# KLab/YAIK

Measured on AMD Instinct MI355X. Metric: Mpix/s tile encode (alpha reject + 7 gradient passes + 8x8 range quant), 8K RGBA, higher is better.
Workload: dtype u8/int32 (+f32 mode-selection sums)

## Files before the change

yaik_amd/csrc/yk_encode2.hip:

```cpp
#include "yk_common.h"
#include "yk_curves.h"
#include "yk_device.h"
#include <mutex>

__constant__ float c_curve2[6][16] = YK_CURVE_TABLE;

#define LS YK_LSTRIDE
#ifdef YK_TEST_HOOKS
#define YK2_ABLATE(bit) ((P.ablate & (bit)) != 0)
#else
#define YK2_ABLATE(bit) false
#endif

__device__ __forceinline__ int y2_byte(uint32_t w, int ch) { return (w >> (8 * ch)) & 255; }
__device__ __forceinline__ uint32_t y2_absdiff(uint32_t a, uint32_t b) { uint32_t r; asm("v_sad_u32 %0, %1, %2, 0" : "=v"(r) : "v"(a), "v"(b)); return r; }
__device__ __forceinline__ int y2_round6(int v) { return (v & ~3) | (v >> 6); }
__device__ __forceinline__ int y2_round6p(int v) { v = min(v + 1, 255); return (v & ~3) | (v >> 6); }

typedef short y2s2 __attribute__((ext_vector_type(2)));
typedef unsigned short y2u2 __attribute__((ext_vector_type(2)));
__device__ __forceinline__ y2u2 y2_u2(uint32_t w) { return __builtin_bit_cast(y2u2, w); }
__device__ __forceinline__ y2s2 y2_s2(y2u2 v) { return __builtin_bit_cast(y2s2, v); }
__device__ __forceinline__ y2u2 y2_splat(int v) { const unsigned short t = (unsigned short)v; return (y2u2){ t, t }; }
__device__ __forceinline__ y2s2 y2_splats(int v) { const short t = (short)v; return (y2s2){ t, t }; }
// ... 283 lines not shown
        const y2s2 rA = __builtin_elementwise_max(__builtin_elementwise_sub_sat(W.loR, mnA), __builtin_elementwise_sub_sat(mxA, W.hiR));
        unsigned long long f = y2_fold<NX, NY>(__ballot(oA.x > 0));
        f &= y2_fold<NX, NY>(__ballot(oA.y > 0));
        f &= y2_fold<NX, NY>(__ballot(rA.x > 0));
        f &= y2_fold<NX, NY>(__ballot(rA.y > 0));
        return f;
    };
    auto failP2 = [&](const y2s2 mnP, const y2s2 mxP) -> unsigned long long {
        const y2s2 oP = __builtin_elementwise_max(__builtin_elementwise_sub_sat(W.loO, mnP), __builtin_elementwise_sub_sat(mxP, W.hiO));
        const y2s2 rP = __builtin_elementwise_max(__builtin_elementwise_sub_sat(W.loR, mnP), __builtin_elementwise_sub_sat(mxP, W.hiR));
        return y2_fold<NX, NY>(__ballot((oP.x > 0) | (oP.y > 0))) & y2_fold<NX, NY>(__ballot((rP.x > 0) | (rP.y > 0)));
    };
    auto mnAll = [&]() { return __builtin_elementwise_min(__builtin_elementwise_min(mn[0], mn[1]), mn[2]); };
    auto mxAll = [&]() { return __builtin_elementwise_max(__builtin_elementwise_max(mx[0], mx[1]), mx[2]); };

    constexpr bool kScreen = (NX * NY >= 4);
    constexpr unsigned kA = 0x07u, kP = 0x18u;
    unsigned long long accept;
    if (SMOOTH) {
        setup(0); setup(1); setup(2);
        pixelRow(0, kA, true);
        nextRow(0, kA); pixelRow(1, kA, false);
        nextRow(1, kA); pixelRow(2, kA, false);
        nextRow(2, kA); pixelRow(3, kA, false);
        YK2_STAT(kPassId * 10 + 4, 1);
        accept = viable & ~failA4(mnAll(), mxAll());
        const unsigned long long rest = viable & ~accept;
        if (rest != 0ULL) {
            YK2_STAT(kPassId * 10 + 5, 1); YK2_STAT(90 + kPassId, __popcll(y2_spread<NX, NY>(rest)));
            setup(3);
            pixelRow(0, 0x08u, true);
            const unsigned long long left = rest & ~failP2(mn[3], mx[3]);
            if (left != 0ULL) {
                setup(4);
                pixelRow(0, 0x10u, true);
                nextRow(0, kP); pixelRow(1, kP, false);
                nextRow(1, kP); pixelRow(2, kP, false);
                nextRow(2, kP); pixelRow(3, kP, false);
                accept |= left & ~failP2(__builtin_elementwise_min(mn[3], mn[4]), __builtin_elementwise_max(mx[3], mx[4]));
            }
        }
    } else {
        if (kScreen) {
            setup(0); setup(3);
            pixelRow(0, 0x09u, true);
            viable &= ~(failA4(mn[0], mx[0]) & failP2(mn[3], mx[3]));
            if (viable == 0ULL) { YK2_STAT(kPassId * 10 + 2, 1); return 0ULL; }
            setup(1); setup(2);
            pixelRow(0, 0x06u, true);
            viable &= ~(failA4(mnAll(), mxAll()) & failP2(mn[3], mx[3]));
            if (viable == 0ULL) { YK2_STAT(kPassId * 10 + 3, 1); return 0ULL; }
            nextRow(0, kA);
            pixelRow(1, kA, false);
        } else {
#pragma unroll
            for (int t = 0; t < 5; t++) setup(t);
            pixelRow(0, 0x1Fu, true);
            viable &= ~(failA4(mnAll(), mxAll()) & failP2(__builtin_elementwise_min(mn[3], mn[4]), __builtin_elementwise_max(mx[3], mx[4])));
            if (viable == 0ULL) { YK2_STAT(kPassId * 10 + 3, 1); return 0ULL; }
            nextRow(0, 0x1Fu);
            pixelRow(1, 0x1Fu, false);
            if (NX * NY <= 2) {
                viable &= ~(failA4(mnAll(), mxAll()) & failP2(__builtin_elementwise_min(mn[3], mn[4]), __builtin_elementwise_max(mx[3], mx[4])));
                if (viable == 0ULL) { YK2_STAT(kPassId * 10 + 9, 1); return 0ULL; }
            }
        }
        YK2_STAT(kPassId * 10 + 4, 1);
        nextRow(1, kA);
        pixelRow(2, kA, false);
        nextRow(2, kA);
        pixelRow(3, kA, false);
        accept = viable & ~failA4(mnAll(), mxAll());
        const unsigned long long rest = viable & ~accept;
        if (rest != 0ULL) {
            YK2_STAT(kPassId * 10 + 5, 1); YK2_STAT(90 + kPassId, __popcll(y2_spread<NX, NY>(rest)));
            if (kScreen) {
                setup(4);
                pixelRow(0, 0x10u, true);
                nextRow(0, kP);
                pixelRow(1, kP, false);
            }
            nextRow(1, kP);
            pixelRow(2, kP, false);
            nextRow(2, kP);
            pixelRow(3, kP, false);
            accept |= rest & ~failP2(__builtin_elementwise_min(mn[3], mn[4]), __builtin_elementwise_max(mx[3], mx[4]));
        }
    }
    return accept;
}

template <int SX, int SY, bool SMOOTH = false>
__device__ __forceinline__ void y2_grad_pass(const Y2Pass pass, unsigned long long& cov, unsigned long long& evaluated) {
    constexpr int NX = (1 << SX) / 4, NY = (1 << SY) / 4, kPassId = y2_pass_id<SX, SY>();
    const int lane = pass.lane;
    const unsigned long long viable = y2_viable<SX, SY>(pass, cov) & ~evaluated;
    evaluated = 0ULL;
    if (viable == 0ULL) return;
    YK2_STAT(kPassId * 10 + 0, 1); YK2_STAT(kPassId * 10 + 8, __popcll(y2_spread<NX, NY>(viable)));
    if (y2_compact_sweep<SX, SY>(pass, viable, cov, evaluated)) return;
    const unsigned long long accept = y2_full_pass<SX, SY, SMOOTH>(pass, viable);
    if (accept == 0ULL) return;
    YK2_STAT(kPassId * 10 + 6, 1);
    y2_accept<SX, SY>(pass, cov, accept);
}

#define YK2_QROWS 258
#define YK2_QR0 32
#define YK2_QNR 224
#define YK2_QBYTES ((size_t)YK2_QNR * YK2_QROWS * 16)
#define YK2_RCPBYTES ((size_t)256 * sizeof(float))
#define YK2_DEFN1 224
#define YK2_DEFBYTES ((size_t)225 * YK2_DEFN1 * 4)
#define YK2_TABBYTES (YK2_QBYTES + YK2_RCPBYTES + YK2_DEFBYTES)
typedef _Float16 y2h2 __attribute__((ext_vector_type(2)));
__device__ __forceinline__ uint32_t y2_f16_bits(int n) { const _Float16 h = (_Float16)(float)n; return (uint32_t)__builtin_bit_cast(unsigned short, h); }
__global__ void yk_qtab_kernel(uint4* tab) {
    __shared__ int K[6][16];
    const int R = YK2_QR0 + (int)blockIdx.x, t = threadIdx.x;
    if (t < 96) { const int m = t >> 4, i = t & 15; K[m][i] = __float2int_rz(__fmul_rn(c_curve2[m][i], (float)R)); }
    __syncthreads();
    if (t < YK2_QROWS) {
        const int o = t - 2;
        uint32_t md[6], idx = 0;
        for (int m = 0; m < 6; m++) {
            const int cnt = m < 3 ? 16 : 8;
            int best = 1 << 30, bi = 0;
            for (int n = 0; n < cnt; n++) { const int d = abs(K[m][n] - o); if (d < best) { best = d; bi = n; } }
            best = min(best, 255);
            md[m] = y2_f16_bits(best);
            idx |= (uint32_t)bi << (4 * m);
        }
        tab[(size_t)blockIdx.x * YK2_QROWS + t] = make_uint4(md[0] | (md[1] << 16), md[2] | (md[3] << 16), md[4] | (md[5] << 16), idx);
    }
}
struct Y2TileDef { int base, BN, dist, R; };
__device__ __forceinline__ Y2TileDef y2_tile_def(const int min_, const int d8) {
    Y2TileDef d;
    d.base = (min_ * 63 + 112) / 224;
    d.BN = (d.base * 224) / 63;
    const int scale = 223 - d.BN;
    const int dnum = (d8 - 32) * 127 + (scale - 1);
    d.dist = (scale < 0) ? -dnum : dnum / scale;
    d.R = (d.dist * scale) / 127 + 32;
    return d;
}
__global__ void yk_deftab_kernel(uint32_t* tab) {
    const int min_ = blockIdx.x, d8 = 32 + (int)threadIdx.x;
    const Y2TileDef d = y2_tile_def(min_, d8);
    const int R = min(max(d.R, YK2_QR0), YK2_QR0 + YK2_QNR - 1);
    const uint32_t rowBase = (uint32_t)((R - YK2_QR0) * YK2_QROWS + 2 - d.BN + 256);
    tab[min_ * YK2_DEFN1 + (int)threadIdx.x] = rowBase | (((((uint32_t)d.dist & 255u) << 7) | ((uint32_t)d.base & 255u)) << 16);
}

__global__ void yk_selftest_qtab_kernel(const uint4* tab, const uint32_t* deftab, int* mismatches) {
    const int mn = blockIdx.x, mx = threadIdx.x;
    if (mx < mn) return;
    const int min_ = min(mn, 224);
    int diff = mx - min_; if (diff < 16) diff = 16;
    const int d8 = max(diff, 32);
    const Y2TileDef d = y2_tile_def(min_, d8);
    const int BN = d.BN, R = d.R;
    int bad = 0;
    if (R < YK2_QR0 || R >= YK2_QR0 + YK2_QNR || mn - BN < -2) { atomicAdd(mismatches, 1); return; }
    {
        const uint32_t e = deftab[min_ * YK2_DEFN1 + (d8 - 32)];
        if ((e & 0xFFFFu) != (uint32_t)((R - YK2_QR0) * YK2_QROWS + 2 - BN + 256)) bad++;
        if ((e >> 16) != ((((uint32_t)d.dist & 255u) << 7) | ((uint32_t)d.base & 255u))) bad++;
    }
    for (int m = 0; m < 6; m++) {
        const int cnt = m < 3 ? 16 : 8;
        int L[16];
        for (int i = 0; i < cnt; i++) {
            L[i] = __float2int_rz(__fadd_rn((float)BN, __fmul_rn(c_curve2[m][i], (float)R)));
            if (L[i] != BN + __float2int_rz(__fmul_rn(c_curve2[m][i], (float)R))) bad++;
        }
        for (int v = mn; v <= mx; v++) {
            int best = 1 << 30, bi = 0;
            for (int n = 0; n < cnt; n++) { const int dd = abs(L[n] - v); if (dd < best) { best = dd; bi = n; } }
            const uint4 row = tab[(size_t)(R - YK2_QR0) * YK2_QROWS + (v - BN + 2)];
            const uint32_t w = m < 2 ? row.x : (m < 4 ? row.y : row.z);
            const uint32_t hb = (m & 1) ? (w >> 16) : (w & 0xFFFFu);
            const int ix = (row.w >> (4 * m)) & 15;
            if (hb != y2_f16_bits(best) || ix != bi) bad++;
        }
    }
    if (bad) atomicAdd(mismatches, bad);
}

#define YK2_RUN 16
template <int K> __device__ __forceinline__ uint32_t y2_writelane_k(uint32_t v, uint32_t old) { asm("v_writelane_b32 %0, %1, %2" : "+v"(old) : "s"(v), "n"(K)); return old; }
__device__ __forceinline__ uint32_t y2_writelane(uint32_t v, int k, uint32_t old) {
    switch (k) {
        case 0: return y2_writelane_k<0>(v, old); case 1: return y2_writelane_k<1>(v, old); case 2: return y2_writelane_k<2>(v, old);
        case 3: return y2_writelane_k<3>(v, old); case 4: return y2_writelane_k<4>(v, old); case 5: return y2_writelane_k<5>(v, old);
        case 11: return y2_writelane_k<11>(v, old); default: return y2_writelane_k<12>(v, old);
    }
}
#ifdef YK2_TIMING
__device__ unsigned long long g_y2_times[65536 * 16];
#define YK2_PROBE(i) do { if ((i) == 0 && lane == 0 && unit < 65536) { g_y2_times[(size_t)unit * 16 + 10] = 0; g_y2_times[(size_t)unit * 16 + 11] = 0; g_y2_times[(size_t)unit * 16 + 12] = y2_t_entry; g_y2_times[(size_t)unit * 16 + 13] = ((unsigned long long)y2_xcc << 32) | y2_hwid; } if (lane == 0 && unit < 65536) { g_y2_times[(size_t)unit * 16 + 2 * (i)] = __builtin_amdgcn_s_memtime(); g_y2_times[(size_t)unit * 16 + 2 * (i) + 1] = __builtin_amdgcn_s_memrealtime(); } } while (0)
extern "C" int yk_debug_wave_times(unsigned long long* out) { return (int)hipMemcpyFromSymbol(out, HIP_SYMBOL(g_y2_times), sizeof(g_y2_times)); }
#else
#define YK2_PROBE(i) do { } while (0)
#endif
#define YK2_LUTW 84
#ifndef YK2_WIN
#define YK2_WIN 16
#endif
#ifndef YK2_PREF
#define YK2_PREF 8
#endif
#ifndef YK2_RVWIN
#define YK2_RVWIN 8
#endif

#define Y2_QUAD_X 0xB1
#define Y2_QUAD_Y 0x4E
template <int CTRL> __device__ __forceinline__ int y2_quad(int v) { return __builtin_amdgcn_update_dpp(v, v, CTRL, 0xF, 0xF, true); }
template <int CTRL> __device__ __forceinline__ float y2_quad(float v) { return __int_as_float(y2_quad<CTRL>(__float_as_int(v))); }
template <int FIRST> __device__ __forceinline__ void y2_quad_sums(float (&t)[6]) {
#define Y2_QX(i) "v_add_f32_dpp %" #i ", %" #i ", %" #i " quad_perm:[1,0,3,2] row_mask:0xf bank_mask:0xf\n\t"
#define Y2_QY(i) "v_add_f32_dpp %" #i ", %" #i ", %" #i " quad_perm:[2,3,0,1] row_mask:0xf bank_mask:0xf\n\t"
    if (FIRST == 0)
        asm volatile("s_nop 1\n\t" Y2_QX(0) Y2_QX(1) Y2_QX(2) Y2_QX(3) Y2_QX(4) Y2_QX(5) Y2_QY(0) Y2_QY(1) Y2_QY(2) Y2_QY(3) Y2_QY(4) Y2_QY(5)
                     : "+v"(t[0]), "+v"(t[1]), "+v"(t[2]), "+v"(t[3]), "+v"(t[4]), "+v"(t[5]));
    else
        asm volatile("s_nop 1\n\t" Y2_QX(0) Y2_QX(1) Y2_QX(2) Y2_QY(0) Y2_QY(1) Y2_QY(2) : "+v"(t[3]), "+v"(t[4]), "+v"(t[5]));
#undef Y2_QX
#undef Y2_QY
}
__device__ __forceinline__ float y2_row16_sum(float x) {
    x = __fadd_rn(x, y2_quad<Y2_QUAD_X>(x));
    x = __fadd_rn(x, y2_quad<Y2_QUAD_Y>(x));
    x = __fadd_rn(x, __int_as_float(__builtin_amdgcn_update_dpp(0, __float_as_int(x), 0x141, 0xF, 0xF, true)));
    x = __fadd_rn(x, __int_as_float(__builtin_amdgcn_update_dpp(0, __float_as_int(x), 0x140, 0xF, 0xF, true)));
    return x;
}
__device__ __forceinline__ uint32_t y2_byte_x4(uint32_t w, int ch) {
    uint32_t r; const uint32_t two = 2u;
    if (ch == 0) asm("v_lshlrev_b32_sdwa %0, %1, %2 dst_sel:DWORD dst_unused:UNUSED_PAD src0_sel:DWORD src1_sel:BYTE_0" : "=v"(r) : "v"(two), "v"(w));
    else if (ch == 1) asm("v_lshlrev_b32_sdwa %0, %1, %2 dst_sel:DWORD dst_unused:UNUSED_PAD src0_sel:DWORD src1_sel:BYTE_1" : "=v"(r) : "v"(two), "v"(w));
    else asm("v_lshlrev_b32_sdwa %0, %1, %2 dst_sel:DWORD dst_unused:UNUSED_PAD src0_sel:DWORD src1_sel:BYTE_2" : "=v"(r) : "v"(two), "v"(w));
    return r;
}
__device__ __forceinline__ void y2_fma_lo(float& acc, uint32_t h, float w) { asm volatile("v_fma_mix_f32 %0, %1, %2, %0 op_sel_hi:[1,0,0]" : "+v"(acc) : "v"(h), "v"(w)); }
__device__ __forceinline__ void y2_fma_hi(float& acc, uint32_t h, float w) { asm volatile("v_fma_mix_f32 %0, %1, %2, %0 op_sel:[1,0,0] op_sel_hi:[1,0,0]" : "+v"(acc) : "v"(h), "v"(w)); }
__device__ __forceinline__ uint32_t y2_pack3(int r, int g, int b) {
    return __builtin_amdgcn_perm((uint32_t)b, __builtin_amdgcn_perm((uint32_t)g, (uint32_t)r, 0x0C0C0400u), 0x0C040100u);
}

template <bool WANT_DST, bool MODE3>
__global__ __launch_bounds__(64, 4) void yk_encode2_kernel(const YkEncodeParams P) {
    constexpr int kStart = MODE3 ? 3 : 0;
    constexpr int kPixWords = 17 * LS, kLutWords = WANT_DST ? 16 * YK2_LUTW : 0;
    __shared__ __attribute__((aligned(16))) uint32_t s_mem[kPixWords > kLutWords ? kPixWords : kLutWords];
    uint32_t* const s_pix = s_mem;
    uint32_t (*const s_lut)[YK2_LUTW] = reinterpret_cast<uint32_t (*)[YK2_LUTW]>(s_mem);
    __shared__ uint32_t s_bm[24];
    __shared__ uint8_t s_list[64];
    __shared__ __attribute__((aligned(16))) float s_curve[WANT_DST ? 6 : 1][16];
    __shared__ __attribute__((aligned(16))) float s_rcp[256];
    __shared__ __attribute__((aligned(16))) uint32_t s_aux[432];
    uint32_t* const s_lat = s_aux;
    float (*const s_chain)[68] = reinterpret_cast<float (*)[68]>(s_aux);
    float* const s_err = reinterpret_cast<float*>(s_aux + 408);
    __shared__ uint32_t s_range[3 * 64];
    __shared__ __attribute__((aligned(16))) uint32_t s_sp[3 * 4 * 8 + 3 * 4 * 16];

    uint32_t* const s_tile = s_aux + 416;
    __shared__ uint32_t s_iwTest[WANT_DST ? 1024 : 1];
    uint32_t* const s_iw = WANT_DST ? s_iwTest : s_mem;
    uint32_t* const s_park = WANT_DST ? s_iwTest : s_sp;
    static_assert(WANT_DST || kPixWords >= 1024, "index words need 4 KB");

    const int lane = threadIdx.x;
    __builtin_amdgcn_s_setprio(3);
#ifdef YK2_TIMING
    const unsigned long long y2_t_entry = __builtin_amdgcn_s_memrealtime();
    const unsigned y2_hwid = __builtin_amdgcn_s_getreg((4 << 0) | (0 << 6) | (31 << 11)), y2_xcc = __builtin_amdgcn_s_getreg((20 << 0) | (0 << 6) | (31 << 11));
#endif
    typedef const __attribute__((address_space(4))) YkEncodeParams* Y2ParamPtr;
    auto strip = [&](const int slot, const int xcd, const int lane, Y2ParamPtr const Pp) {
    const __attribute__((address_space(4))) YkEncodeParams& P = *Pp;
    const int nBf = P.xBB64 * P.yBB64, nB = nBf * P.nFrames;
    const int grp = slot / (YK2_RUN * 4);
    const int unit = (grp * 8 + ((xcd + grp) & 7)) * (YK2_RUN * 4) + (slot - grp * (YK2_RUN * 4));
    int L = unit >> 2; const int wave = unit & 3;
    const bool spare = L >= nB;
    L = spare ? 0 : L;
    const uint32_t frU = yk_udiv((uint32_t)L, P.divNBf.mul, P.divNBf.shift);
    L -= (int)frU * nBf;
    const size_t fr = frU;
    const int32_t* const pl0 = P.plane[0] + fr * P.fs.plane; const int32_t* const pl1 = P.plane[1] + fr * P.fs.plane; const int32_t* const pl2 = P.plane[2] + fr * P.fs.plane;
    const int BY = (int)yk_udiv((uint32_t)L, P.divXBB64.mul, P.divXBB64.shift), BX = L - BY * P.xBB64;
    const int w = P.w, h = P.h;
    const int mt0 = (BY * 4 + wave) * P.mtW + BX * 4;

    YK2_PROBE(0);
    if (lane < 24) s_bm[lane] = 0;
    typedef uint32_t y2_u32x2 __attribute__((ext_vector_type(2)));
    typedef int32_t y2_i32x4 __attribute__((ext_vector_type(4)));
    y2_u32x2 keep8; y2_i32x4 bnd;
    {
        const int g4 = (lane & 15) * 4, r0 = lane >> 4;
        const int gx = BX * 64 + g4;
        const bool inX = gx + 3 < w;
        const int gxc = min(gx, w - 4);
        const int gyS = BY * 64 + wave * 16;
        const int gyB = min(gyS, P.hAvail - 1);
        const size_t rowBase = (size_t)gyB * (size_t)P.strideElems;
        const char* const b0 = reinterpret_cast<const char*>(pl0 + rowBase);
        const char* const b1 = reinterpret_cast<const char*>(pl1 + rowBase);
        const char* const b2 = reinterpret_cast<const char*>(pl2 + rowBase);
        int4 R[4], G[4], B[4];
#pragma unroll
        for (int k = 0; k < 4; k++) {
            const int rel = min(gyS + r0 + 4 * k, P.hAvail - 1) - gyB;
            const uint32_t off = (uint32_t)(rel * P.strideElems + gxc) * 4u;
            R[k] = *reinterpret_cast<const int4*>(b0 + off);
            G[k] = *reinterpret_cast<const int4*>(b1 + off);
            B[k] = *reinterpret_cast<const int4*>(b2 + off);
        }
        int4 Rb, Gb, Bb;
        {
            const int rel = min(gyS + 16, P.hAvail - 1) - gyB;
            const uint32_t off = (uint32_t)(rel * P.strideElems + gxc) * 4u;
            Rb = *reinterpret_cast<const int4*>(b0 + off);
            Gb = *reinterpret_cast<const int4*>(b1 + off);
            Bb = *reinterpret_cast<const int4*>(b2 + off);
        }
        uint32_t hcol;
        const int hr = min(max(lane - 32, 0), 16);
        {
            const int rel = min(gyS + hr, P.hAvail - 1) - gyB;
            const uint32_t off = (uint32_t)(rel * P.strideElems + min(BX * 64 + 64, w - 1)) * 4u;
            hcol = y2_pack3(*reinterpret_cast<const int32_t*>(b0 + off), *reinterpret_cast<const int32_t*>(b1 + off), *reinterpret_cast<const int32_t*>(b2 + off));
        }
        const float4 rc4 = *reinterpret_cast<const float4*>(P.qtab + YK2_QBYTES + (size_t)lane * 16);
        const uint4* const orow = P.outTab + (wave * YK2_OT_ROWS + (lane & (YK2_OT_ROWS - 1))) * 2;
        const uint4 ta = orow[0], tb = orow[1];
        {
            const bool rowIn = BY * 64 + wave * 16 < h;
            const uintptr_t args = reinterpret_cast<uintptr_t>(Pp);
            const uintptr_t kpIn = reinterpret_cast<uintptr_t>(P.keep) + fr * P.fs.keep + (uintptr_t)(mt0 & ~3);
            const uintptr_t bpIn = reinterpret_cast<uintptr_t>(P.bounds) + fr * 64;
            const uintptr_t kp = (P.keep != nullptr && rowIn) ? kpIn : args, bp = P.bounds != nullptr ? bpIn : args;
            asm volatile("s_load_dwordx2 %0, %2, 0x0\n\ts_load_dwordx4 %1, %3, 0x0" : "=&s"(keep8), "=&s"(bnd) : "s"(kp), "s"(bp));
        }

        __builtin_amdgcn_s_setprio(0);
        if (spare) return;
        {
            const uint32_t frT = frU + P.outFrame0;
            const uint32_t o = ta.x + frT * ta.y + (uint32_t)BX * ta.z + (uint32_t)BY * ta.w;
            s_park[lane] = ((uint32_t)BX < tb.x && (uint32_t)BY < tb.y) ? o : YK2_OT_NONE;
            s_park[64 + lane] = tb.z;
        }
        uint4 o[4], ob;
#pragma unroll
        for (int k = 0; k < 4; k++) {
            o[k] = make_uint4(y2_pack3(R[k].x, G[k].x, B[k].x), y2_pack3(R[k].y, G[k].y, B[k].y), y2_pack3(R[k].z, G[k].z, B[k].z), y2_pack3(R[k].w, G[k].w, B[k].w));
            *reinterpret_cast<uint4*>(&s_pix[(r0 + 4 * k) * LS + g4]) = o[k];
        }
        ob = make_uint4(y2_pack3(Rb.x, Gb.x, Bb.x), y2_pack3(Rb.y, Gb.y, Bb.y), y2_pack3(Rb.z, Gb.z, Bb.z), y2_pack3(Rb.w, Gb.w, Bb.w));
        if (lane < 16) *reinterpret_cast<uint4*>(&s_pix[16 * LS + g4]) = ob;
        if (BX * 64 + 64 > w) {
            if (!inX) {
#pragma unroll
                for (int k = 0; k < 4; k++) *reinterpret_cast<uint4*>(&s_pix[(r0 + 4 * k) * LS + g4]) = make_uint4(o[k].w, o[k].w, o[k].w, o[k].w);
                if (lane < 16) *reinterpret_cast<uint4*>(&s_pix[16 * LS + g4]) = make_uint4(ob.w, ob.w, ob.w, ob.w);
            }
        }
        if (lane >= 32 && lane <= 48) s_pix[hr * LS + 64] = hcol;
        *reinterpret_cast<float4*>(&s_rcp[lane * 4]) = rc4;

    }
    asm volatile("s_waitcnt lgkmcnt(0)" : "+s"(keep8), "+s"(bnd));
    __syncthreads();
    YK2_PROBE(1);

    const int q = lane >> 4, cx = y2_cell_x(lane & 15), cy = y2_cell_y(lane & 15);
    const int bxCell = q * 16 + cx * 4, byCell = wave * 16 + cy * 4;
    const int gxCell = BX * 64 + bxCell, gyCell = BY * 64 + byCell;
    const int lcell = (cy * 4) * LS + bxCell;
    const int lat = cy * 17 + q * 4 + cx;
    const bool mtIn = (BX * 64 + q * 16 < w) && (BY * 64 + wave * 16 < h);

    uint32_t pw[16];
#pragma unroll
    for (int r = 0; r < 4; r++) {
        const uint4 t = *reinterpret_cast<const uint4*>(&s_pix[lcell + r * LS]);
        pw[r * 4 + 0] = t.x; pw[r * 4 + 1] = t.y; pw[r * 4 + 2] = t.z; pw[r * 4 + 3] = t.w;
    }

    unsigned long long cov = 0ULL;
    unsigned long long evaluated = 0ULL;
    {
        bool dead = !mtIn;
        {
            const int lim = 4 * P.rejectFactor + 1;
            const y2u2 rb0 = y2_u2(pw[0] & 0x00FF00FFu), rb1 = y2_u2(pw[1] & 0x00FF00FFu), rb2 = y2_u2(pw[2] & 0x00FF00FFu), rb3 = y2_u2(pw[3] & 0x00FF00FFu);
            const y2u2 ga = y2_u2(__builtin_amdgcn_perm(pw[1], pw[0], 0x0C050C01u)), gb = y2_u2(__builtin_amdgcn_perm(pw[2], pw[1], 0x0C050C01u)),
                       gc = y2_u2(__builtin_amdgcn_perm(pw[3], pw[2], 0x0C050C01u));
            const y2u2 l2 = y2_splat(lim);
            const y2u2 u1 = rb0 + rb2 - rb1 - rb1 + l2, u2 = rb1 + rb3 - rb2 - rb2 + l2, ug = ga + gc - gb - gb + l2;
            const y2u2 um = __builtin_elementwise_max(__builtin_elementwise_max(u1, u2), ug);
            dead |= __builtin_bit_cast(uint32_t, __builtin_elementwise_sub_sat(um, y2_splat(2 * lim))) != 0u;
        }
        const unsigned long long deadLanes = __ballot(dead);
        YK2_STAT(75, 1); YK2_STAT(76, ~deadLanes == 0ULL ? 1 : 0); YK2_STAT(77, __popcll(deadLanes));
        const bool stripInside = (BX * 64 + 64 <= w) && (BY * 64 + wave * 16 + 16 <= h);
        if (~deadLanes != 0ULL && !YK2_ABLATE(2)) {
            auto latticePoint = [&](const int idx) {
                const int lr = (idx * 241) >> 12, lc = idx - lr * 17;
                const uint32_t raw = s_pix[(lr * 4) * LS + lc * 4];
                const uint32_t r6 = (raw & 0x00FCFCFCu) | ((raw >> 6) & 0x00030303u);
                const uint32_t z = (raw & 0x007F7F7Fu) + 0x00010101u;
                const uint32_t inc = (z ^ (raw & 0x00808080u)) | (((z & raw & 0x00808080u) >> 7) * 255u);
                const uint32_t p6 = (inc & 0x00FCFCFCu) | ((inc >> 6) & 0x00030303u);
                s_lat[0 * YK2_LATN + idx] = __builtin_amdgcn_perm(r6, raw, 0x0C040C00u);
                s_lat[1 * YK2_LATN + idx] = __builtin_amdgcn_perm(r6, raw, 0x0C050C01u);
                s_lat[2 * YK2_LATN + idx] = __builtin_amdgcn_perm(r6, raw, 0x0C060C02u);
                s_lat[3 * YK2_LATN + idx] = __builtin_amdgcn_perm(p6, p6, 0x0C010C00u);
                s_lat[4 * YK2_LATN + idx] = __builtin_amdgcn_perm(p6, p6, 0x0C020C02u);
            };
            latticePoint(lane);
            if (lane < YK2_LATN - 64) latticePoint(lane + 64);
            __syncthreads();
            y2s2 rg[16], bb[8];
#pragma unroll
            for (int k = 0; k < 16; k++) rg[k] = y2_rg(pw[k]);
#pragma unroll
            for (int k = 0; k < 8; k++) bb[k] = y2_bb(pw[2 * k], pw[2 * k + 1]);
            const Y2Pass S = { s_lat, lat, cx, cy, rg, bb, deadLanes, stripInside, gxCell, gyCell, w, h, P.rejectFactor, s_bm, bxCell, byCell, s_pix, s_list, s_range, lane };
            if (deadLanes == 0ULL) y2_grad_pass<4, 4, true>(S, cov, evaluated);
            else y2_grad_pass<4, 4>(S, cov, evaluated);
            if (~(cov | deadLanes) != 0ULL) {
                y2_grad_pass<4, 3>(S, cov, evaluated);
                y2_grad_pass<3, 4>(S, cov, evaluated);
                y2_grad_pass<3, 3>(S, cov, evaluated);
                y2_grad_pass<3, 2>(S, cov, evaluated);
                y2_grad_pass<2, 3>(S, cov, evaluated);
                y2_grad_pass<2, 2>(S, cov, evaluated);
            }
#pragma unroll
            for (int r = 0; r < 4; r++) {
                const uint4 t = *reinterpret_cast<const uint4*>(&s_pix[lcell + r * LS]);
                pw[r * 4 + 0] = t.x; pw[r * 4 + 1] = t.y; pw[r * 4 + 2] = t.z; pw[r * 4 + 3] = t.w;
            }
        }
    }
    const int mtIdx = mt0 + q;
    __syncthreads();
    YK2_PROBE(2);
    uint8_t* const small = P.small;
    const uint32_t tabOff = s_park[lane], tabSel = s_park[64 + lane];
    const uint32_t tabVal = (s_bm[tabSel & 31u] >> ((tabSel >> 8) & 31u)) & (~0u >> (tabSel >> 16));
    uint32_t off32 = (uint32_t)lane - 8u < 5u ? tabOff : ~0u;
    uint32_t val32 = (uint32_t)lane - 8u < 3u ? tabVal : 0u;
    {
        if ((uint32_t)lane - 1u < 3u) *(small + tabOff) = (uint8_t)tabVal;
        const unsigned long long t = ((cov >> 2) ^ cov) & 0x0C0C0C0C0C0C0C0CULL;
        const unsigned long long covRM = cov ^ t ^ (t << 2);
        uint32_t off16 = ((lane & 15) == 0 && mtIn) ? P.oCov + (frU * (uint32_t)P.fs.coverage + (uint32_t)mtIdx) * 2u : ~0u;
        uint32_t val16 = (uint32_t)((covRM >> (q * 16)) & 0xFFFFULL);
        if ((uint32_t)lane - 4u < 3u) { off16 = tabOff; val16 = tabVal; }
        if (off16 != ~0u) *reinterpret_cast<uint16_t*>(small + off16) = (uint16_t)val16;
        if (P.pixCache != nullptr) {
            const bool cellIn = (gxCell < w) && (gyCell < h);
            if (cellIn && !((cov >> lane) & 1ULL)) {
                const uint32_t strip = (uint32_t)((BY * 4 + wave) * P.xBB64 + BX);
                uint4* dstp = P.pixCache + (size_t)strip * 256 + lane;
#pragma unroll
                for (int r = 0; r < 4; r++) dstp[r * 64] = make_uint4(pw[r * 4 + 0], pw[r * 4 + 1], pw[r * 4 + 2], pw[r * 4 + 3]);
            }
        }
    }
    YK2_PROBE(3);
    int cxB = 0, cyB = 0, cw = w, chh = P.fullH, discard = 1;
    if (P.bounds != nullptr) {
        const int b0 = bnd.x, b1 = bnd.y, b2 = bnd.z, b3 = bnd.w;
        discard = (b0 == 0 && b1 == 0 && b2 == w && b3 == P.fullH) ? 1 : 0;
        cxB = (b0 >> 3) << 3; cyB = (b1 >> 3) << 3;
        cw = (((b2 + 7) >> 3) << 3) - cxB; chh = (((b3 + 7) >> 3) << 3) - cyB;
    }
    const int cxl = cx & 1, cyl = cy & 1;
    const int tgx = gxCell - cxl * 4, tgyl = gyCell - cyl * 4, tgy = tgyl + P.y0;
    const bool tileIn = (tgx + 8 <= w) && (tgyl + 8 <= h);
    const bool part = tileIn && tgx >= cxB && tgx < cxB + cw && tgy >= cyB && tgy < cyB + chh && (tgx + 8 <= cw) && (tgy + 8 <= chh);
    const uint32_t keep4 = (uint32_t)((((unsigned long long)keep8.y << 32) | keep8.x) >> (8 * (mt0 & 3)));
    const bool keepMT = (P.keep == nullptr) || discard || (mtIn && ((keep4 >> (8 * q)) & 0xFFu) != 0u);
    const bool tileLive = part && keepMT;
    const int l00 = lane & ~3;
    const uint32_t quadN = (uint32_t)((~cov) >> l00) & 15u;
    const int v00 = (int)(quadN & 1u), v01 = (int)((quadN >> 2) & 1u);
    const bool valid = tileLive && ((quadN >> (lane & 3)) & 1u);
    const int nTop = __popc(quadN & 3u), nBot = __popc(quadN >> 2);
    const int tileIdx = (tgyl >> 3) * P.tilesW + (tgx >> 3);
    const size_t T8 = (size_t)P.tilesW * P.tilesH;
    const int tw = lane >> 2;
    const bool writer = ((lane & 3) == 0) && tileIn;
    const unsigned long long validMask = __ballot(valid);
    const bool fullTiles = !WANT_DST && __ballot(tileLive && quadN != 15u && quadN != 0u) == 0ULL;

    {
        const int n16 = (tileLive && !YK2_ABLATE(1)) ? (nTop + nBot) : 0;
        if ((P.tilesW & 7) == 0) {
            if (validMask != 0ULL) {
#pragma unroll
                for (int r = 0; r < 2; r++) {
                    const bool mine = writer && ((cy >> 1) == r);
                    const unsigned long long b0 = __ballot(mine && (n16 & 1)), b1 = __ballot(mine && (n16 & 2)), b2 = __ballot(mine && (n16 & 4));
                    const unsigned long long bd = __ballot(mine && n16 > 0);
                    val32 = y2_writelane((uint32_t)(__popcll(b0) + 2 * __popcll(b1) + 4 * __popcll(b2)) | ((uint32_t)__popcll(bd) << 16), 11 + r, val32);
                }
            }
        } else if (writer && n16 > 0) {
            uint32_t* const blockCntP = P.blockCnt + fr * P.fs.blockN;
            atomicAdd(&blockCntP[((size_t)tileIdx >> 10) * 2], 16u * (uint32_t)n16);
            atomicAdd(&blockCntP[((size_t)tileIdx >> 10) * 2 + 1], 1u);
        }
        if (off32 != ~0u) *reinterpret_cast<uint32_t*>(small + off32) = val32;
    }

    YK2_STAT(70, validMask != 0ULL ? 1 : 0); YK2_STAT(74, __popcll(validMask));
    { const int nv = __popcll(validMask); YK2_STAT(120 + (nv == 0 ? 0 : nv <= 4 ? 1 : nv <= 8 ? 2 : nv <= 16 ? 3 : nv <= 32 ? 4 : nv < 64 ? 5 : 6), 1); (void)nv; }
    uint32_t defs01 = 0u, defs2c = 0u;
    if (validMask != 0ULL && !YK2_ABLATE(1)) {
        uint8_t* const slotsP = P.slots + fr * P.fs.slots;
        uint32_t* lut = &s_lut[WANT_DST ? tw : 0][0];
        if (WANT_DST) {
            s_curve[lane >> 4][lane & 15] = c_curve2[lane >> 4][lane & 15];
            if (lane < 32) s_curve[4 + (lane >> 4)][lane & 15] = c_curve2[4 + (lane >> 4)][lane & 15];
        }
        const int j4 = lane & 3;
        const int nValidLanes = __popcll(validMask);
        const bool spread = nValidLanes <= 4 && !WANT_DST;
        const int vRank = (int)__builtin_amdgcn_mbcnt_hi((uint32_t)(validMask >> 32), __builtin_amdgcn_mbcnt_lo((uint32_t)validMask, 0u));
        uint32_t slotOff[4];
#pragma unroll
        for (int r = 0; r < 4; r++) {
            const int yIn = cyl * 4 + r;
            const int pos = (yIn < 4) ? (yIn * 4 * nTop + (cxl ? 4 * v00 : 0))
                                      : (16 * nTop + (yIn - 4) * 4 * nBot + (cxl ? 4 * v01 : 0));
            slotOff[r] = (uint32_t)tileIdx * (uint32_t)YK_SLOT + (uint32_t)(pos >> 1);
        }
        int tmn[3], tmx[3];
        {
            y2u2 mnRB = y2_splat(0xFFFF), mxRB = y2_splat(0), mnG = y2_splat(0xFFFF), mxG = y2_splat(0);
            if (valid) {
#pragma unroll
                for (int k = 0; k < 16; k += 2) {
                    const y2u2 a = y2_u2(pw[k] & 0x00FF00FFu), b = y2_u2(pw[k + 1] & 0x00FF00FFu), g = y2_u2(__builtin_amdgcn_perm(pw[k + 1], pw[k], 0x0C050C01u));
                    if (k == 0) { mnRB = __builtin_elementwise_min(a, b); mxRB = __builtin_elementwise_max(a, b); mnG = g; mxG = g; }
                    else {
                        mnRB = __builtin_elementwise_min(__builtin_elementwise_min(mnRB, a), b); mxRB = __builtin_elementwise_max(__builtin_elementwise_max(mxRB, a), b);
                        mnG = __builtin_elementwise_min(mnG, g); mxG = __builtin_elementwise_max(mxG, g);
                    }
                }
            }
            tmn[0] = (int)mnRB.x; tmn[2] = (int)mnRB.y; tmx[0] = (int)mxRB.x; tmx[2] = (int)mxRB.y;
            tmn[1] = min((int)mnG.x, (int)mnG.y); tmx[1] = max((int)mxG.x, (int)mxG.y);
#pragma unroll
            for (int p = 0; p < 3; p++) {
                tmn[p] = min(tmn[p], y2_quad<Y2_QUAD_X>(tmn[p])); tmx[p] = max(tmx[p], y2_quad<Y2_QUAD_X>(tmx[p]));
                tmn[p] = min(tmn[p], y2_quad<Y2_QUAD_Y>(tmn[p])); tmx[p] = max(tmx[p], y2_quad<Y2_QUAD_Y>(tmx[p]));
            }
        }
        const uint32_t* const defTab = reinterpret_cast<const uint32_t*>(P.qtab + YK2_QBYTES + YK2_RCPBYTES);
        uint32_t tdef[3];
#pragma unroll
        for (int p = 0; p < 3; p++) {
            const int none = tmn[p] > 255;
            const int mn = none ? 0 : tmn[p], mx = none ? 0 : tmx[p];
            const int min_ = min(mn, 224);
            const int d8 = max(mx - min_, 32);
            tdef[p] = defTab[(uint32_t)(min_ * YK2_DEFN1 + d8 - 32)];
            s_range[p * 64 + lane] = (uint32_t)mn | ((uint32_t)mx << 8);
        }
        const uint8_t* const qrows = P.qtab - (size_t)256 * 16;
        if (spread && !YK2_ABLATE(4)) {
            if (valid) s_list[vRank] = (uint8_t)lane;
            __builtin_amdgcn_fence(__ATOMIC_RELEASE, "wavefront"); __builtin_amdgcn_wave_barrier(); __builtin_amdgcn_fence(__ATOMIC_ACQUIRE, "wavefront");
            const int spI = lane >> 4, spK = lane & 15;
            const bool spAct = spI < nValidLanes;
            const int spSrc = (int)s_list[spAct ? spI : 0];
            const int sq = spSrc >> 4, scx = y2_cell_x(spSrc & 15), scy = y2_cell_y(spSrc & 15);
            const uint32_t spx = s_pix[(scy * 4 + (spK >> 2)) * LS + sq * 16 + scx * 4 + (spK & 3)];
#pragma unroll
            for (int p = 0; p < 3; p++) {
                const uint32_t q16s = (uint32_t)__builtin_amdgcn_ds_bpermute(spSrc << 2, (int)((tdef[p] & 0xFFFFu) << 4));
                float t6[6] = { 0.0f, 0.0f, 0.0f, 0.0f, 0.0f, 0.0f };
                if (spAct) {
                    const uint32_t v4 = y2_byte_x4(spx, p);
                    const uint4 row = *reinterpret_cast<const uint4*>(qrows + (size_t)((v4 << 2) + q16s));
                    const float rv = *reinterpret_cast<const float*>(reinterpret_cast<const char*>(s_rcp) + v4);
                    if (!MODE3) { y2_fma_lo(t6[0], row.x, rv); y2_fma_hi(t6[1], row.x, rv); y2_fma_lo(t6[2], row.y, rv); }
                    y2_fma_hi(t6[3], row.y, rv); y2_fma_lo(t6[4], row.z, rv); y2_fma_hi(t6[5], row.z, rv);
                    s_sp[96 + (p * 4 + spI) * 16 + spK] = row.w;
                }
#pragma unroll
                for (int m = kStart; m < 6; m++) {
                    const float tot = y2_row16_sum(t6[m]);
                    if (spK == 0) s_sp[(p * 4 + spI) * 8 + m] = __float_as_uint(tot);
                }
            }
            __builtin_amdgcn_fence(__ATOMIC_RELEASE, "wavefront"); __builtin_amdgcn_wave_barrier(); __builtin_amdgcn_fence(__ATOMIC_ACQUIRE, "wavefront");
        }
        uint4 win[16];
        auto issueRows = [&](const int pl, const int k0, const int k1) {
            if (valid && !spread && !YK2_ABLATE(4)) {
                const uint32_t q16 = (tdef[pl] & 0xFFFFu) << 4;
                {
#pragma unroll
                    for (int k = k0; k < k1; k++) {
                        const uint32_t v4 = y2_byte_x4(pw[k], pl);
                        win[k] = *reinterpret_cast<const uint4*>(qrows + (size_t)((v4 << 2) + q16));
                    }
                }
            }
        };
        issueRows(0, 0, YK2_PREF);
#pragma unroll
        for (int p = 0; p < 3; p++) {
            const uint32_t qrow16 = (tdef[p] & 0xFFFFu) << 4;
            float sm[6] = { 0.0f, 0.0f, 0.0f, 0.0f, 0.0f, 0.0f };
            issueRows(p, YK2_PREF, 16);
            if (valid && !spread && !YK2_ABLATE(4)) {
                float rvw[YK2_RVWIN];
                auto issueRcp = [&](const int k, float& rv) { rv = *reinterpret_cast<const float*>(reinterpret_cast<const char*>(s_rcp) + y2_byte_x4(pw[k], p)); };
#pragma unroll
                for (int k = 0; k < YK2_RVWIN; k++) issueRcp(k, rvw[k]);
#pragma unroll
                for (int k = 0; k < 16; k++) {
                    __builtin_amdgcn_sched_barrier(0);
                    const uint4 row = win[k]; const float rv = rvw[k % YK2_RVWIN];
                    if (!MODE3) { y2_fma_lo(sm[0], row.x, rv); y2_fma_hi(sm[1], row.x, rv); y2_fma_lo(sm[2], row.y, rv); }
                    y2_fma_hi(sm[3], row.y, rv); y2_fma_lo(sm[4], row.z, rv); y2_fma_hi(sm[5], row.z, rv);
                    s_iw[k * 64 + lane] = row.w;
                    if (k + YK2_RVWIN < 16) issueRcp(k + YK2_RVWIN, rvw[k % YK2_RVWIN]);
                }
                __builtin_amdgcn_sched_barrier(0);
            }
            if (spread && valid && !YK2_ABLATE(4)) {
#pragma unroll
                for (int m = kStart; m < 6; m++) sm[m] = __uint_as_float(s_sp[(p * 4 + vRank) * 8 + m]);
#pragma unroll
                for (int k4 = 0; k4 < 4; k4++) {
                    const uint4 iw4 = *reinterpret_cast<const uint4*>(&s_sp[96 + (p * 4 + vRank) * 16 + k4 * 4]);
                    s_iw[(k4 * 4 + 0) * 64 + lane] = iw4.x; s_iw[(k4 * 4 + 1) * 64 + lane] = iw4.y; s_iw[(k4 * 4 + 2) * 64 + lane] = iw4.z; s_iw[(k4 * 4 + 3) * 64 + lane] = iw4.w;
                }
            }
            if (p < 2) issueRows(p + 1, 0, YK2_PREF);
            float tm[6] = { sm[0], sm[1], sm[2], sm[3], sm[4], sm[5] };
            y2_quad_sums<kStart>(tm);
            int bestMode = kStart; float bestT = tm[kStart];
            bool near = false;
#pragma unroll
            for (int m = kStart + 1; m < 6; m++) {
                const float t = tm[m];
                const float lo = fminf(t, bestT), hi = fmaxf(t, bestT);
                near |= !(__fmul_rn(lo, 1.00002f) < hi);
                bestMode = (t <= bestT) ? m : bestMode;
                bestT = lo;
            }
            bool amb = false;
            uint32_t ties = 0;
            if (__ballot(near && tileLive) != 0ULL) {
                int bm = kStart; float bt = tm[kStart];
#pragma unroll
                for (int m = kStart + 1; m < 6; m++) {
                    const float t = tm[m];
                    const float lo = fminf(t, bt), hi = fmaxf(t, bt);
                    const bool eq = (t == bt);
                    amb |= !eq && !(__fmul_rn(lo, 1.00002f) < hi);
                    if (eq && t != 0.0f) ties |= (1u << m) | ((uint32_t)bm << (8 + 3 * m));
                    bm = (t <= bt) ? m : bm;
                    bt = lo;
                }
            }
            if (__ballot(ties != 0u && tileLive) != 0ULL) {
                YK2_STAT(73, 1);
                const uint32_t tr = s_range[p * 64 + lane];
                const uint32_t mn = tr & 255u, mx = tr >> 8;
                const uint32_t va = min(mn + (uint32_t)j4, mx), vb = min(mn + 4u + (uint32_t)j4, mx);
                const uint4 ra = *reinterpret_cast<const uint4*>(qrows + (size_t)((va << 4) + qrow16));
                const uint4 rb = *reinterpret_cast<const uint4*>(qrows + (size_t)((vb << 4) + qrow16));
                const uint32_t rxa = __builtin_amdgcn_alignbit(ra.x, ra.x, 16), rya = __builtin_amdgcn_alignbit(ra.y, ra.y, 16), rza = __builtin_amdgcn_alignbit(ra.z, ra.z, 16);
                const uint32_t rxb = __builtin_amdgcn_alignbit(rb.x, rb.x, 16), ryb = __builtin_amdgcn_alignbit(rb.y, rb.y, 16), rzb = __builtin_amdgcn_alignbit(rb.z, rb.z, 16);
                uint32_t acc[9] = { (ra.x ^ rxa) | (rb.x ^ rxb),
                                    (ra.y ^ rya) | (rb.y ^ ryb),
                                    (ra.z ^ rza) | (rb.z ^ rzb),
                                    (ra.x ^ ra.y) | (rb.x ^ rb.y),
                                    (ra.x ^ ra.z) | (rb.x ^ rb.z),
                                    (ra.y ^ ra.z) | (rb.y ^ rb.z),
                                    (ra.x ^ rya) | (rb.x ^ ryb),
                                    (ra.x ^ rza) | (rb.x ^ rzb),
                                    (ra.y ^ rza) | (rb.y ^ rzb) };
#pragma unroll
                for (int i = 0; i < 9; i++) { acc[i] |= (uint32_t)y2_quad<Y2_QUAD_X>((int)acc[i]); acc[i] |= (uint32_t)y2_quad<Y2_QUAD_Y>((int)acc[i]); }
                bool differ = (mx - mn) > 7u;
                auto pairDiffers = [&](const int i, const int j) -> bool {
                    const int lo = i < j ? i : j, hi = i < j ? j : i;
                    if (lo == 0 && hi == 1) return (acc[0] & 0xFFFFu) != 0u;
                    if (lo == 2 && hi == 3) return (acc[1] & 0xFFFFu) != 0u;
                    if (lo == 4 && hi == 5) return (acc[2] & 0xFFFFu) != 0u;
                    if (lo == 0 && hi == 2) return (acc[3] & 0xFFFFu) != 0u;
                    if (lo == 1 && hi == 3) return (acc[3] >> 16) != 0u;
                    if (lo == 0 && hi == 4) return (acc[4] & 0xFFFFu) != 0u;
                    if (lo == 1 && hi == 5) return (acc[4] >> 16) != 0u;
                    if (lo == 2 && hi == 4) return (acc[5] & 0xFFFFu) != 0u;
                    if (lo == 3 && hi == 5) return (acc[5] >> 16) != 0u;
                    if (lo == 0 && hi == 3) return (acc[6] & 0xFFFFu) != 0u;
                    if (lo == 1 && hi == 2) return (acc[6] >> 16) != 0u;
                    if (lo == 0 && hi == 5) return (acc[7] & 0xFFFFu) != 0u;
                    if (lo == 1 && hi == 4) return (acc[7] >> 16) != 0u;
                    if (lo == 2 && hi == 5) return (acc[8] & 0xFFFFu) != 0u;
                    return (acc[8] >> 16) != 0u;
                };
#pragma unroll
                for (int m = kStart + 1; m < 6; m++) {
                    const uint32_t fb = ((ties >> m) & 1u) ? ((ties >> (8 + 3 * m)) & 7u) : 7u;
#pragma unroll
                    for (int b2 = kStart; b2 < m; b2++) differ |= (fb == (uint32_t)b2) && pairDiffers(b2, m);
                }
                if (ties != 0u && differ) amb = true;
            }
            uint32_t cLo = 0, cHi = 0;
            if (valid) {
                const uint32_t sh = 4u * (uint32_t)bestMode;
#pragma unroll
                for (int k = 0; k < 16; k++) {
                    const uint32_t code = s_iw[k * 64 + lane] >> sh;
                    if (k < 8) cLo = __builtin_amdgcn_alignbit(code, cLo, 4); else cHi = __builtin_amdgcn_alignbit(code, cHi, 4);
                }
            }
            if (YK2_ABLATE(16)) amb = true;
            unsigned long long ambMask = __ballot(amb && tileLive);
            YK2_STAT(72, __popcll(ambMask) / 4); YK2_STAT(71, ambMask != 0ULL ? 1 : 0);
#ifdef YK2_TIMING
            if (lane == 0 && unit < 65536 && ambMask) { g_y2_times[(size_t)unit * 16 + 10] += (unsigned long long)__popcll(ambMask) / 4; g_y2_times[(size_t)unit * 16 + 11] += 1; }
#endif
            if (WANT_DST) {
                const int rowBase = (int)(tdef[p] & 0xFFFFu) - 256 - 2;
                const int base = (int)((tdef[p] >> 16) & 127u);
                const int BN = (base * 224) / 63;
                const int rangeDecode = (rowBase + BN) / YK2_QROWS + YK2_QR0;
                const float Rf = (float)rangeDecode, BNf = (float)BN;
#pragma unroll
                for (int m = 0; m < 3; m++) {
                    uint32_t Lq[4];
#pragma unroll
                    for (int k = 0; k < 4; k++)
                        Lq[k] = (uint32_t)__float2int_rz(__fadd_rn(BNf, __fmul_rn(s_curve[m][j4 * 4 + k], Rf)));
                    *reinterpret_cast<uint4*>(&lut[m * 20 + j4 * 4]) = make_uint4(Lq[0] << 8, Lq[1] << 8, Lq[2] << 8, Lq[3] << 8);
                }
#pragma unroll
                for (int m = 3; m < 6; m++) {
                    uint32_t Lq[2];
#pragma unroll
                    for (int k = 0; k < 2; k++)
                        Lq[k] = (uint32_t)__float2int_rz(__fadd_rn(BNf, __fmul_rn(s_curve[m][j4 * 2 + k], Rf)));
                    *reinterpret_cast<uint2*>(&lut[60 + (m - 3) * 8 + j4 * 2]) = make_uint2(Lq[0] << 8, Lq[1] << 8);
                }
                __builtin_amdgcn_fence(__ATOMIC_RELEASE, "wavefront");
                __builtin_amdgcn_wave_barrier();
                __builtin_amdgcn_fence(__ATOMIC_ACQUIRE, "wavefront");
            }
            while (ambMask != 0ULL) {
                const int a00 = (__ffsll((long long)ambMask) - 1) & ~3;
                ambMask &= ~(0xFULL << a00);
                if (l00 == a00) {
#pragma unroll
                    for (int r = 0; r < 4; r++) {
                        const uint32_t kSel = 0x0C0C0000u | ((4u + (uint32_t)p) << 8) | (uint32_t)p;
                        const uint32_t lo2 = __builtin_amdgcn_perm(pw[r * 4 + 1], pw[r * 4 + 0], kSel), hi2 = __builtin_amdgcn_perm(pw[r * 4 + 3], pw[r * 4 + 2], kSel);
                        s_tile[(cyl * 4 + r) * 2 + cxl] = __builtin_amdgcn_perm(hi2, lo2, 0x05040100u);
                    }
                }
                const uint32_t tq16 = (uint32_t)__builtin_amdgcn_readlane((int)qrow16, a00), tqn = (uint32_t)__builtin_amdgcn_readlane((int)quadN, a00);
                __builtin_amdgcn_fence(__ATOMIC_RELEASE, "wavefront");
                __builtin_amdgcn_wave_barrier();
                __builtin_amdgcn_fence(__ATOMIC_ACQUIRE, "wavefront");
                {
                    const uint32_t v = (uint32_t)reinterpret_cast<const uint8_t*>(s_tile)[lane];
                    const bool pv = ((tqn >> (((lane >> 5) << 1) | ((lane >> 2) & 1))) & 1u) != 0u;
                    uint4 rw = make_uint4(0u, 0u, 0u, 0u);
                    if (pv) rw = *reinterpret_cast<const uint4*>(qrows + (size_t)((v << 4) + tq16));
                    const float fv = (float)v, rr = pv ? s_rcp[v] : 0.0f;
                    const y2h2 h01 = __builtin_bit_cast(y2h2, rw.x), h23 = __builtin_bit_cast(y2h2, rw.y), h45 = __builtin_bit_cast(y2h2, rw.z);
                    s_chain[0][lane] = yk_div_exact((float)h01.x, fv, rr);
                    s_chain[1][lane] = yk_div_exact((float)h01.y, fv, rr);
                    s_chain[2][lane] = yk_div_exact((float)h23.x, fv, rr);
                    s_chain[3][lane] = yk_div_exact((float)h23.y, fv, rr);
                    s_chain[4][lane] = yk_div_exact((float)h45.x, fv, rr);
                    s_chain[5][lane] = yk_div_exact((float)h45.y, fv, rr);
                }
                __builtin_amdgcn_fence(__ATOMIC_RELEASE, "wavefront");
                __builtin_amdgcn_wave_barrier();
                __builtin_amdgcn_fence(__ATOMIC_ACQUIRE, "wavefront");
                if (lane < 6 && lane >= kStart) {
                    float sacc = 0.0f;
                    const float4* cp = reinterpret_cast<const float4*>(&s_chain[lane][0]);
#pragma unroll
                    for (int k = 0; k < 16; k++) {
                        const float4 a = cp[k];
// ... 114 lines not shown
```

Measured before the change: 242,700.

## Skip pixel reload and tile setup when strip cannot produce coded tiles

Computes keep/bounds discard state early and defines a per-wave 'cannot code' condition: the strip is inside the image and every cell is covered, or the keep mask rejects the whole strip. When it holds, the kernel skips reloading the 4x4 pixel words from LDS after the gradient passes and skips the tile-liveness, ballot and bounds computation in the tail. The bottom halo row is also loaded as one dword per lane instead of int4 per 16 lanes, which removes the edge-replication store. The change adds branching and a new path that must stay equivalent to the old tile liveness logic. The keep-mask semantics also change: keepMT no longer treats a null keep pointer as keep-all and relies on discard defaulting to 1.

```diff
diff --git a/yaik_amd/csrc/yk_encode2.hip b/yaik_amd/csrc/yk_encode2.hip
--- a/yaik_amd/csrc/yk_encode2.hip
+++ b/yaik_amd/csrc/yk_encode2.hip
@@ -609,6 +609,7 @@
     typedef uint32_t y2_u32x2 __attribute__((ext_vector_type(2)));
     typedef int32_t y2_i32x4 __attribute__((ext_vector_type(4)));
     y2_u32x2 keep8; y2_i32x4 bnd;
+    int fullH = P.fullH;
     {
         const int g4 = (lane & 15) * 4, r0 = lane >> 4;
         const int gx = BX * 64 + g4;
@@ -629,13 +630,13 @@
             G[k] = *reinterpret_cast<const int4*>(b1 + off);
             B[k] = *reinterpret_cast<const int4*>(b2 + off);
         }
-        int4 Rb, Gb, Bb;
+        int32_t Rb, Gb, Bb;
         {
             const int rel = min(gyS + 16, P.hAvail - 1) - gyB;
-            const uint32_t off = (uint32_t)(rel * P.strideElems + gxc) * 4u;
-            Rb = *reinterpret_cast<const int4*>(b0 + off);
-            Gb = *reinterpret_cast<const int4*>(b1 + off);
-            Bb = *reinterpret_cast<const int4*>(b2 + off);
+            const uint32_t off = (uint32_t)(rel * P.strideElems + min(BX * 64 + lane, w - 1)) * 4u;
+            Rb = *reinterpret_cast<const int32_t*>(b0 + off);
+            Gb = *reinterpret_cast<const int32_t*>(b1 + off);
+            Bb = *reinterpret_cast<const int32_t*>(b2 + off);
         }
         uint32_t hcol;
         const int hr = min(max(lane - 32, 0), 16);
@@ -654,6 +655,7 @@
             const uintptr_t bpIn = reinterpret_cast<uintptr_t>(P.bounds) + fr * 64;
             const uintptr_t kp = (P.keep != nullptr && rowIn) ? kpIn : args, bp = P.bounds != nullptr ? bpIn : args;
             asm volatile("s_load_dwordx2 %0, %2, 0x0\n\ts_load_dwordx4 %1, %3, 0x0" : "=&s"(keep8), "=&s"(bnd) : "s"(kp), "s"(bp));
+            asm volatile("" : "+s"(fullH));
         }
 
         __builtin_amdgcn_s_setprio(0);
@@ -664,19 +666,17 @@
             s_park[lane] = ((uint32_t)BX < tb.x && (uint32_t)BY < tb.y) ? o : YK2_OT_NONE;
             s_park[64 + lane] = tb.z;
         }
-        uint4 o[4], ob;
+        uint4 o[4];
 #pragma unroll
         for (int k = 0; k < 4; k++) {
             o[k] = make_uint4(y2_pack3(R[k].x, G[k].x, B[k].x), y2_pack3(R[k].y, G[k].y, B[k].y), y2_pack3(R[k].z, G[k].z, B[k].z), y2_pack3(R[k].w, G[k].w, B[k].w));
             *reinterpret_cast<uint4*>(&s_pix[(r0 + 4 * k) * LS + g4]) = o[k];
         }
-        ob = make_uint4(y2_pack3(Rb.x, Gb.x, Bb.x), y2_pack3(Rb.y, Gb.y, Bb.y), y2_pack3(Rb.z, Gb.z, Bb.z), y2_pack3(Rb.w, Gb.w, Bb.w));
-        if (lane < 16) *reinterpret_cast<uint4*>(&s_pix[16 * LS + g4]) = ob;
+        s_pix[16 * LS + lane] = y2_pack3(Rb, Gb, Bb);
         if (BX * 64 + 64 > w) {
             if (!inX) {
 #pragma unroll
                 for (int k = 0; k < 4; k++) *reinterpret_cast<uint4*>(&s_pix[(r0 + 4 * k) * LS + g4]) = make_uint4(o[k].w, o[k].w, o[k].w, o[k].w);
-                if (lane < 16) *reinterpret_cast<uint4*>(&s_pix[16 * LS + g4]) = make_uint4(ob.w, ob.w, ob.w, ob.w);
             }
         }
         if (lane >= 32 && lane <= 48) s_pix[hr * LS + 64] = hcol;
@@ -703,6 +703,13 @@
 
     unsigned long long cov = 0ULL;
     unsigned long long evaluated = 0ULL;
+    int discard = 1; uint32_t keep4 = 0u; bool allRejected = false;
+    if (P.keep != nullptr) {
+        discard = ((P.bounds == nullptr) | ((uint32_t)(bnd.x | bnd.y | (bnd.z ^ w) | (bnd.w ^ fullH)) == 0u)) ? 1 : 0;
+        keep4 = (uint32_t)((((unsigned long long)keep8.y << 32) | keep8.x) >> (8 * (mt0 & 3)));
+        allRejected = !discard & (keep4 == 0u);
+    }
+    bool shortTail = false;
     {
         bool dead = !mtIn;
         {
@@ -718,6 +725,7 @@
         const unsigned long long deadLanes = __ballot(dead);
         YK2_STAT(75, 1); YK2_STAT(76, ~deadLanes == 0ULL ? 1 : 0); YK2_STAT(77, __popcll(deadLanes));
         const bool stripInside = (BX * 64 + 64 <= w) && (BY * 64 + wave * 16 + 16 <= h);
+        auto cannotCode = [&](const unsigned long long covered) { return (stripInside && ~covered == 0ULL) || allRejected; };
         if (~deadLanes != 0ULL && !YK2_ABLATE(2)) {
             auto latticePoint = [&](const int idx) {
                 const int lr = (idx * 241) >> 12, lc = idx - lr * 17;
@@ -751,12 +759,18 @@
                 y2_grad_pass<2, 3>(S, cov, evaluated);
                 y2_grad_pass<2, 2>(S, cov, evaluated);
             }
-#pragma unroll
-            for (int r = 0; r < 4; r++) {
-                const uint4 t = *reinterpret_cast<const uint4*>(&s_pix[lcell + r * LS]);
-                pw[r * 4 + 0] = t.x; pw[r * 4 + 1] = t.y; pw[r * 4 + 2] = t.z; pw[r * 4 + 3] = t.w;
-            }
-        }
+            if (!cannotCode(cov) || (~cov != 0ULL && P.pixCache != nullptr)) {
+#pragma unroll
+                for (int r = 0; r < 4; r++) {
+                    const uint4 t = *reinterpret_cast<const uint4*>(&s_pix[lcell + r * LS]);
+                    pw[r * 4 + 0] = t.x; pw[r * 4 + 1] = t.y; pw[r * 4 + 2] = t.z; pw[r * 4 + 3] = t.w;
+                }
+            } else {
+#pragma unroll
+                for (int k = 0; k < 16; k++) asm volatile("" : "=v"(pw[k]));
+            }
+        }
+        shortTail = cannotCode(cov);
     }
     const int mtIdx = mt0 + q;
     __syncthreads();
@@ -785,31 +799,37 @@
         }
     }
     YK2_PROBE(3);
-    int cxB = 0, cyB = 0, cw = w, chh = P.fullH, discard = 1;
-    if (P.bounds != nullptr) {
-        const int b0 = bnd.x, b1 = bnd.y, b2 = bnd.z, b3 = bnd.w;
-        discard = (b0 == 0 && b1 == 0 && b2 == w && b3 == P.fullH) ? 1 : 0;
-        cxB = (b0 >> 3) << 3; cyB = (b1 >> 3) << 3;
-        cw = (((b2 + 7) >> 3) << 3) - cxB; chh = (((b3 + 7) >> 3) << 3) - cyB;
-    }
     const int cxl = cx & 1, cyl = cy & 1;
     const int tgx = gxCell - cxl * 4, tgyl = gyCell - cyl * 4, tgy = tgyl + P.y0;
     const bool tileIn = (tgx + 8 <= w) && (tgyl + 8 <= h);
-    const bool part = tileIn && tgx >= cxB && tgx < cxB + cw && tgy >= cyB && tgy < cyB + chh && (tgx + 8 <= cw) && (tgy + 8 <= chh);
-    const uint32_t keep4 = (uint32_t)((((unsigned long long)keep8.y << 32) | keep8.x) >> (8 * (mt0 & 3)));
-    const bool keepMT = (P.keep == nullptr) || discard || (mtIn && ((keep4 >> (8 * q)) & 0xFFu) != 0u);
-    const bool tileLive = part && keepMT;
     const int l00 = lane & ~3;
-    const uint32_t quadN = (uint32_t)((~cov) >> l00) & 15u;
-    const int v00 = (int)(quadN & 1u), v01 = (int)((quadN >> 2) & 1u);
-    const bool valid = tileLive && ((quadN >> (lane & 3)) & 1u);
-    const int nTop = __popc(quadN & 3u), nBot = __popc(quadN >> 2);
     const int tileIdx = (tgyl >> 3) * P.tilesW + (tgx >> 3);
     const size_t T8 = (size_t)P.tilesW * P.tilesH;
     const int tw = lane >> 2;
     const bool writer = ((lane & 3) == 0) && tileIn;
-    const unsigned long long validMask = __ballot(valid);
-    const bool fullTiles = !WANT_DST && __ballot(tileLive && quadN != 15u && quadN != 0u) == 0ULL;
+    bool tileLive = false, valid = false, fullTiles = !WANT_DST;
+    uint32_t quadN = 0u;
+    int v00 = 0, v01 = 0, nTop = 0, nBot = 0;
+    unsigned long long validMask = 0ULL;
+    if (shortTail) {
+        YK2_STAT(78, 1);
+    } else {
+        int cxB = 0, cyB = 0, cw = w, chh = P.fullH;
+        if (P.bounds != nullptr) {
+            const int b0 = bnd.x, b1 = bnd.y, b2 = bnd.z, b3 = bnd.w;
+            cxB = (b0 >> 3) << 3; cyB = (b1 >> 3) << 3;
+            cw = (((b2 + 7) >> 3) << 3) - cxB; chh = (((b3 + 7) >> 3) << 3) - cyB;
+        }
+        const bool part = tileIn && tgx >= cxB && tgx < cxB + cw && tgy >= cyB && tgy < cyB + chh && (tgx + 8 <= cw) && (tgy + 8 <= chh);
+        const bool keepMT = discard || (mtIn && ((keep4 >> (8 * q)) & 0xFFu) != 0u);
+        tileLive = part && keepMT;
+        quadN = (uint32_t)((~cov) >> l00) & 15u;
+        v00 = (int)(quadN & 1u); v01 = (int)((quadN >> 2) & 1u);
+        valid = tileLive && ((quadN >> (lane & 3)) & 1u);
+        nTop = __popc(quadN & 3u); nBot = __popc(quadN >> 2);
+        validMask = __ballot(valid);
+        fullTiles = !WANT_DST && __ballot(tileLive && quadN != 15u && quadN != 0u) == 0ULL;
+    }
 
     {
         const int n16 = (tileLive && !YK2_ABLATE(1)) ? (nTop + nBot) : 0;
```

Result: faster. 245,200, median of 5 (+1.0%).
